# AugmentariumLab/VolumeRenderer

Measured on AMD Instinct MI355X. Metric: Mvoxels/s kd-tree compress+decode, higher is better.
Workload: dtype u8; 1 GPU; 2048x2048x1920 uint8 volume per GPU as 960 bricks of 256x256x128, rm_volume, tolerance 1, maxEpochs 2, VolumeKdtree build + levelCut

## Files before the change

volumerenderer_amd/csrc/brickset.h:

```cpp
#pragma once
#include "kd_common.h"
#include "../../include/vrhip.h"
#include <algorithm>
#include <string>
#include <vector>

namespace vr {

struct Stream2 {
    uint8_t *temp = nullptr;
    uint8_t *codes = nullptr;
    uint8_t *recon[3] = {nullptr, nullptr, nullptr};
    Ctrl *ctrl = nullptr;
    uint8_t *tree = nullptr;
    uint8_t *treeCompact = nullptr;
};

struct Switches {
    bool decodeWalk = false;
    bool decodeFineV1 = false;
    bool decodeQuad = false;
    bool noSkipBlocks = false;
    bool noUniformBlocks = false;
};

#define VR_LOD_SLOTS 4
struct LodSlot {
    int32_t *dev = nullptr;
    int32_t *host = nullptr;
    uint8_t *idxValCut = nullptr;
    uint32_t *decTables = nullptr;
    uint8_t *rankVals = nullptr;
    int64_t *obDev = nullptr;
    int64_t *obHost = nullptr;
    vr_pool_entry *tabHost = nullptr;
    int64_t tabCap = 0;
    hipEvent_t done = nullptr;
    bool pending = false;
};

struct BrickSet {
    int32_t B = 0;
    Switches sw;
    Geom g{};
    TilePlan tile{};
    RegionPlan region{};
    Pyr12Plan pyr12{};
    int32_t D = 0, maxDepth = 0;
    int32_t tolerance = 6, maxEpochs = 5, variant = 0;
    int32_t K = 0;
    int32_t Ds = 0;
    int64_t heapStride = 0;
    int64_t leafStride = 0;
    int64_t codeStride = 0;
    int64_t reconStride = 0;
    bool leafless = false;
    int64_t treeCap = 0;
    int64_t nIdx = 0;

    Stream2 mid, rng;
    uint8_t *mmMin[2] = {nullptr, nullptr}, *mmMax[2] = {nullptr, nullptr};
    unsigned long long *blockErr = nullptr;
    int64_t nErrBlk = 0;
    void *estSumm = nullptr;
    int64_t estSummStride = 0;
    unsigned long long *blockL1 = nullptr;
    uint8_t *blockFlag = nullptr;
    uint8_t *blockFlagR = nullptr;
    uint8_t *blockAlive = nullptr, *blockVal = nullptr;
    unsigned long long *blockSpine = nullptr, *blockSpineR = nullptr;
    uint32_t *chainLut = nullptr;
    uint32_t *blockTot = nullptr, *blockOff = nullptr;
    bool idx64 = false;
    unsigned long long *blockOff64 = nullptr, *idxBase = nullptr;
    int64_t nEmitBlk = 0;
    uint32_t *idxOff = nullptr;
    uint8_t *idxVal = nullptr;
    uint8_t *idxValCut = nullptr;
    uint8_t *fineIdx = nullptr;
    std::vector<uint8_t> fineHas;
    bool fineAll = false;
    uint32_t *decTables = nullptr;
    uint8_t *idxVal3 = nullptr;
    uint32_t *chainTab = nullptr;
    bool chainTabReady = false;
    std::vector<std::vector<uint8_t>> hostTree;
    uint32_t *lut = nullptr;
    bool foreignRange = false;
    uint32_t *spread = nullptr;
    bool generalGeom = false;
    uint32_t *srcIdx = nullptr;
    uint32_t *ownerRank = nullptr;
    uint8_t *ownerSurv = nullptr;
    uint8_t *rankVals = nullptr;

    std::vector<Ctrl> hostCtrl;
    std::vector<int32_t> hostRevertsR;
    uint32_t lutZeroRun = 0;
    bool encoderReady = false;
    bool built = false, hostCtrlValid = false;
    bool gapped = false;
    bool compactValid = false;
    bool compactOnBuild = true;
    int64_t compactCap = 0;
    unsigned long long *brickOff = nullptr;
    int32_t *compactOverflow = nullptr;
    std::vector<unsigned long long> hostBrickOff;
    bool foreign = false;
    std::vector<int64_t> openTreeBytes;
    hipEvent_t ev[8] = {nullptr, nullptr, nullptr, nullptr, nullptr, nullptr, nullptr, nullptr};
    hipStream_t aux = nullptr, auxN[3] = {nullptr, nullptr, nullptr};
    hipEvent_t evFork = nullptr, evJoin = nullptr, evJoinN[3] = {nullptr, nullptr, nullptr};
    int levelLoopStreams = 2;
    unsigned long long *blockErrR = nullptr;
    void *estSummR = nullptr;
    float phasesMs[5] = {0, 0, 0, 0, 0};
// ... 36 lines not shown
```

volumerenderer_amd/csrc/capi.hip:

```cpp
#include "../../include/vrhip.h"
#include "brickset.h"
#include "raymarch.h"
#include <math.h>
#include <stdio.h>
#include <stdlib.h>
#include <string.h>
#include <algorithm>
#include <array>
#include <atomic>
#include <map>
#include <mutex>
#include <new>

using namespace vr;

struct vr_brickset { BrickSet s; };

#define HIPCHK(x) do { hipError_t e_ = (x); if (e_ != hipSuccess) return e_ == hipErrorOutOfMemory ? VR_ERR_OOM : VR_ERR_NO_DEVICE; } while (0)

static bool device_ok()
{
    int n = 0;
    hipError_t e = hipGetDeviceCount(&n);
    if ((e != hipSuccess || n <= 0) && getenv("VRHIP_DEBUG"))
// ... 143 lines not shown
    HIPCHK(hipMalloc(&b.blockAlive, B * (size_t)b.nEmitBlk));
    HIPCHK(hipMalloc(&b.blockVal, B * (size_t)b.nEmitBlk));
    HIPCHK(hipMalloc(&b.blockSpine, B * (size_t)b.nEmitBlk * sizeof(unsigned long long)));
    if (b.variant == VR_VARIANT_MIDRANGE) HIPCHK(hipMalloc(&b.blockSpineR, B * (size_t)b.nEmitBlk * sizeof(unsigned long long)));
    HIPCHK(hipMalloc(&b.chainLut, (260 + 512) * sizeof(uint32_t)));
    HIPCHK(hipMalloc(&b.blockTot, B * (size_t)b.nEmitBlk * sizeof(uint32_t)));
    HIPCHK(hipMalloc(&b.blockOff, B * (size_t)b.nEmitBlk * sizeof(uint32_t)));
    if (b.idx64) {
        HIPCHK(hipMalloc(&b.blockOff64, B * (size_t)b.nEmitBlk * sizeof(unsigned long long)));
        if (!b.idxBase) HIPCHK(hipMalloc(&b.idxBase, B * (size_t)b.nEmitBlk * sizeof(unsigned long long)));
    }
    return VR_OK;
}

static vr_status ensure_encoder_buffers(BrickSet &b)
{
    if (b.encoderReady) return VR_OK;
    const vr_status rc = alloc_encoder_buffers(b);
    if (rc != VR_OK) { (void)hipGetLastError(); free_encoder_buffers(b); return rc; }
    b.encoderReady = true;
    return VR_OK;
}

vr_status vr_brickset_destroy(vr_brickset *h)
{
    if (!h) return VR_OK;
    BrickSet &b = h->s;
    free_lod_slots(&b);
    hipFree(b.errTable);
    free_encoder_buffers(b);
    free_stream2(b.mid);
    free_stream2(b.rng);
    hipFree(b.brickOff); hipFree(b.compactOverflow);
    hipFree(b.idxOff); hipFree(b.idxVal); hipFree(b.idxValCut); hipFree(b.fineIdx); hipFree(b.idxVal3); hipFree(b.chainTab); hipFree(b.decTables); hipFree(b.lut); hipFree(b.spread); hipFree(b.srcIdx); hipFree(b.ownerRank); hipFree(b.ownerSurv); hipFree(b.rankVals);
    for (int i = 0; i < 8; ++i) if (b.ev[i]) hipEventDestroy(b.ev[i]);
    if (b.evFork) hipEventDestroy(b.evFork);
    for (int i = 0; i < 3; ++i) { if (b.evJoinN[i]) hipEventDestroy(b.evJoinN[i]); if (b.auxN[i]) hipStreamDestroy(b.auxN[i]); }
    delete h;
    return VR_OK;
}

static bool pow2(int64_t v) { return v > 0 && (v & (v - 1)) == 0; }

static bool misaligned16(const void *p) { return ((uintptr_t)p & 15) != 0; }

vr_status vr_brickset_create(vr_brickset **out, int32_t num_bricks, const int64_t dims[3], int32_t tolerance,
                             int32_t max_epochs, int32_t variant)
{
    if (!out || !dims || num_bricks <= 0) return VR_ERR_INVALID;
    if (tolerance < 0 || max_epochs < 0 || variant < 0 || variant > 2) return VR_ERR_INVALID;
    for (int k = 0; k < 3; ++k) if (dims[k] <= 0) return VR_ERR_INVALID;
    bool general = !pow2(dims[0]) || !pow2(dims[1]) || !pow2(dims[2]) || dims[0] > 1024 || dims[1] > 1024 || dims[2] > 1024;
    if (dims[0] > (1ll << 20) || dims[1] > (1ll << 20) || dims[2] > (1ll << 20) || dims[0] * dims[1] * dims[2] >= (1ll << 32))
        return VR_ERR_UNSUPPORTED;
    if (!device_ok()) return VR_ERR_NO_DEVICE;
    vr_brickset *h = new (std::nothrow) vr_brickset();
    if (!h) return VR_ERR_OOM;
    BrickSet &b = h->s;
    b.B = num_bricks;
    {
        Switches &w = b.sw;
        w.decodeWalk = getenv("VRHIP_DECODE_WALK") != nullptr;
        w.decodeFineV1 = getenv("VRHIP_DECODE_FINE_V1") != nullptr;
        w.decodeQuad = getenv("VRHIP_DECODE_QUAD") != nullptr;
        w.noSkipBlocks = getenv("VRHIP_NO_SKIP_BLOCKS") != nullptr;
        w.noUniformBlocks = getenv("VRHIP_NO_UNIFORM_BLOCKS") != nullptr;
    }
    make_geom(b.g, dims);
    b.D = b.g.D;
    if (b.D > 31) { delete h; return VR_ERR_UNSUPPORTED; }
    b.idx64 = b.D > 28 || (getenv("VRHIP_FORCE_IDX64") && b.D >= 12);
    if (b.idx64) general = true;
    if (b.idx64 && num_bricks != 1 && b.D > 28) { delete h; return VR_ERR_UNSUPPORTED; }
    b.generalGeom = general;
    b.maxDepth = b.D + VR_CHAIN_LEVELS;
    b.tolerance = tolerance; b.maxEpochs = max_epochs; b.variant = variant;
    b.K = b.D < 6 ? b.D : 6;
    b.Ds = b.D - b.K;
    b.heapStride = (int64_t)1 << (b.D + 1);
    b.leafStride = (int64_t)1 << b.D;
    b.codeStride = ((b.heapStride + 15) / 16) * 4;
    b.reconStride = b.leafStride;
    const int64_t numMax = b.heapStride - 1 + VR_CHAIN_LEVELS * b.leafStride;
    b.treeCap = ((numMax + 15) / 16 + 2) * 4 + 256;
    if (b.D >= 12) {
        const int64_t gappedBytes = ((int64_t)1 << (b.D - 12)) * 2320 * 4 + 256;
        if (gappedBytes > b.treeCap) b.treeCap = gappedBytes;
    }
    b.nIdx = (int64_t)1 << b.Ds;
    make_plans(b.g, b.K, b.generalGeom, b.idx64, b.treeCap, b.tile, b.region, b.pyr12);
    vr_status rc = alloc_stream2(b, b.mid);
    if (rc == VR_OK) {
        hipError_t e = hipMalloc(&b.idxOff, (size_t)b.B * b.nIdx * sizeof(uint32_t));
        if (e == hipSuccess) e = hipMalloc(&b.idxVal, (size_t)b.B * b.nIdx);
        if (e == hipSuccess) e = hipMalloc(&b.idxValCut, (size_t)b.B * b.nIdx);
        if (e == hipSuccess && general) {
            const int grc = build_general_geometry(&b);
            if (grc != 0) e = grc == -3 ? hipErrorOutOfMemory : hipErrorUnknown;
        }
        const auto upload = [](uint32_t *dst, const std::vector<uint32_t> &v) {
            return hipMemcpy(dst, v.data(), v.size() * sizeof(uint32_t), hipMemcpyHostToDevice);
        };
        if (e == hipSuccess) e = hipMalloc(&b.lut, ((size_t)1 << b.K) * sizeof(uint32_t));
        if (e == hipSuccess && !general) e = upload(b.lut, make_lut(b.g, b.K));
        if (e == hipSuccess && !general) e = hipMalloc(&b.spread, (size_t)(b.g.X + b.g.Y + b.g.Z) * sizeof(uint32_t));
        if (e == hipSuccess && !general) e = upload(b.spread, make_spread(b.g));
        for (int i = 0; i < 8 && e == hipSuccess; ++i) e = hipEventCreate(&b.ev[i]);
        if (e != hipSuccess) rc = e == hipErrorOutOfMemory ? VR_ERR_OOM : VR_ERR_NO_DEVICE;
    }
    if (rc != VR_OK) { vr_brickset_destroy(h); return rc; }
    b.hostCtrl.resize(b.B);
    b.openTreeBytes.assign(b.B, -1);
    *out = h;
    return VR_OK;
}

vr_status vr_brickset_set_switch(vr_brickset *h, const char *name, int32_t value)
{
    if (!h || !name) return VR_ERR_INVALID;
    Switches &w = h->s.sw;
    const bool on = value != 0;
    if (!strcmp(name, "decode_walk")) w.decodeWalk = on;
    else if (!strcmp(name, "decode_fine_v1")) w.decodeFineV1 = on;
    else if (!strcmp(name, "decode_quad")) w.decodeQuad = on;
    else if (!strcmp(name, "no_skip_blocks")) w.noSkipBlocks = on;
    else if (!strcmp(name, "no_uniform_blocks")) w.noUniformBlocks = on;
    else return VR_ERR_INVALID;
    return VR_OK;
}

vr_status vr_brickset_set_compaction(vr_brickset *h, int32_t on_build)
{
    if (!h) return VR_ERR_INVALID;
    h->s.compactOnBuild = on_build != 0;
    return VR_OK;
}

vr_status vr_debug_set(const char *name, int32_t value)
{
    if (!name) return VR_ERR_INVALID;
    if (!strcmp(name, "skip_grid_v1")) { vr::g_skipGridV1.store(value ? 1 : 0); return VR_OK; }
    if (!strcmp(name, "reslice_tile_w")) {
        if (value != 8 && value != 16 && value != 64) return VR_ERR_INVALID;
        vr::g_resliceTileLog2.store(value == 8 ? 3 : (value == 16 ? 4 : 6));
        return VR_OK;
    }
    if (!strcmp(name, "hist_plain")) { vr::g_histPlain.store(value ? 1 : 0); return VR_OK; }
    return VR_ERR_INVALID;
}

vr_status vr_brickset_set_error_tolerance(vr_brickset *h, int32_t tol)
{
    if (!h || tol < 0) return VR_ERR_INVALID;
    h->s.tolerance = tol;
    return VR_OK;
}
vr_status vr_brickset_set_max_epochs(vr_brickset *h, int32_t e)
{
    if (!h || e < 0) return VR_ERR_INVALID;
// ... 1008 lines not shown
```

volumerenderer_amd/csrc/kd_decode.hip:

```cpp
#include "brickset.h"
#include <stdio.h>
#include <algorithm>
#include <stdlib.h>
#include <string.h>

namespace vr {

int launch_status(const char *what)
{
    hipError_t e = hipGetLastError();
    if (e == hipSuccess) return 0;
    if (getenv("VRHIP_DEBUG")) fprintf(stderr, "[vrhip] %s: %s\n", what, hipGetErrorString(e));
    return -1;
}

struct Box3 { int lo[3], hi[3]; };
__device__ __forceinline__ int split_axis(const Box3 &b, int depth, bool &more)
{
    const long long e0 = b.hi[0] - b.lo[0], e1 = b.hi[1] - b.lo[1], e2 = b.hi[2] - b.lo[2];
    more = e0 * e1 * e2 > 1;
    int sd = depth % 3, i = 0;
    while (more && (b.hi[sd] - b.lo[sd]) == 1) sd = (depth + ++i) % 3;
    return sd;
}
// ... 938 lines not shown
#define RG_REGX (16 * RG_WAVES)
#define RG_BLK_WORDS 1028
#define RG_RING_MASK (RG_NP * 256 - 1)
static_assert(RG_REGX == VR_RG_REGX, "region_plan (host_plan.cpp) lays the regions out for this x extent");
static_assert(RG_NP >= 4 && (RG_NP & (RG_NP - 1)) == 0, "the side-cars of the next region are staged in ring slots 2 and 3: at least four pieces, a power of two");

struct RegionArgs {
    const uint8_t *tree;
    int64_t treeCap;
    const uint32_t *idxOff;
    const uint8_t *idxVal;
    const uint8_t *fine;
    const uint8_t *val3;
    int64_t nIdx;
    const Ctrl *ctrls;
    uint8_t *out;
    const uint32_t *spread;
    int X, Y;
    int64_t voxels;
    int D, cut;
    int lrx, lry;
    int jx;
    uint32_t lanePos;
    uint32_t parkP[4];
    uint32_t parkS;
    uint32_t gAddr[4];
    uint32_t gByte;
    uint32_t gOut[8];
    uint32_t xRead[2];
    uint32_t blkX, blkY, blkZ;
    int nreg;
    const int32_t *list, *cuts;
    const int64_t *obase;
};

__device__ __forceinline__ uint32_t wave_incl_scan_max_dpp(uint32_t v)
{
    v = max(v, dpp_u32<0x111, 0xf>(0, v));
    v = max(v, dpp_u32<0x112, 0xf>(0, v));
    v = max(v, dpp_u32<0x114, 0xf>(0, v));
    v = max(v, dpp_u32<0x118, 0xf>(0, v));
    v = max(v, dpp_u32<0x142, 0xa>(0, v));
    v = max(v, dpp_u32<0x143, 0xc>(0, v));
    return v;
}

__device__ __forceinline__ void rg_barrier()
{
    asm volatile("s_waitcnt lgkmcnt(0)\n\ts_barrier" ::: "memory");
}

struct RegionShared {
    uint32_t leafA[1024];
    uint32_t chainB[64];
    int d4[4], d5[4];
    uint32_t buf[RG_WAVES * RG_BLK_WORDS];
    uint32_t ring[RG_WAVES][RG_NP * 256 + 4];
};

__device__ __forceinline__ uint32_t rg_pair(uint32_t y, uint32_t yh, uint32_t dead3, int Vp, const RegionShared &sm, uint32_t &used)
{
    const uint32_t c5 = (y & 3u) | dead3;
    const int V5 = med3i(Vp + *(const int *)((const char *)sm.d5 + (c5 << 2)), 0, 255);
    const bool pr = c5 == 3u;
    const uint32_t keep = pr ? 0u : ~0u;
    const uint32_t yl1 = y >> 2;
// ... 24 lines not shown
{
    const uint32_t b = (pw >> 7) & 30u;
    const int V3 = (int)(pw & 255u);
    const uint32_t dead = ((pw >> 24) & 1u) - 1u;
    const uint32_t lo = __builtin_amdgcn_alignbit(w1, w0, b), hi = __builtin_amdgcn_alignbit(w2, w1, b),
                   hh = __builtin_amdgcn_alignbit(w3, w2, b);
    const uint32_t c4 = __builtin_amdgcn_ubfe(lo, p0, 2) | (dead & 3u);
    const int V4 = med3i(V3 + *(const int *)((const char *)sm.d4 + (c4 << 2)), 0, 255);
    const uint32_t dead3 = c4 == 3u ? 3u : 0u;
    uint32_t used1, used2;
    const uint32_t b01 = rg_pair(__builtin_amdgcn_alignbit(hi, lo, p1), __builtin_amdgcn_alignbit(hh, hi, p1), dead3, V4, sm, used1);
    const uint32_t p2 = p1 + used1;
    const bool q = p2 >= 32u;
    const uint32_t A_ = q ? hi : lo, B_ = q ? hh : hi, C_ = q ? 0u : hh;
    const uint32_t b23 = rg_pair(__builtin_amdgcn_alignbit(B_, A_, p2), __builtin_amdgcn_alignbit(C_, B_, p2), dead3, V4, sm, used2);
    return b01 | (b23 << 16);
}

__device__ __forceinline__ void rg_vm_wait(uint32_t n)
{
    switch (n < 24u ? n : 24u) {
#define RG_W(k) case k: asm volatile("s_waitcnt vmcnt(" #k ")" ::: "memory"); break;
    RG_W(0) RG_W(1) RG_W(2) RG_W(3) RG_W(4) RG_W(5) RG_W(6) RG_W(7) RG_W(8) RG_W(9) RG_W(10) RG_W(11) RG_W(12)
    RG_W(13) RG_W(14) RG_W(15) RG_W(16) RG_W(17) RG_W(18) RG_W(19) RG_W(20) RG_W(21) RG_W(22) RG_W(23) RG_W(24)
#undef RG_W
    }
}

#define RG_DMA(SUFFIX, gptr, ldsByte) do { uint32_t keep_; \
    asm volatile("s_mov_b32 %0, m0\n\ts_mov_b32 m0, %2\n\ts_nop 0\n\tglobal_load_lds_" SUFFIX " %1, off\n\ts_mov_b32 m0, %0" \
                 : "=&s"(keep_) : "v"(gptr), "s"(ldsByte) : "memory"); } while (0)

#define RG_IDXD 3

__global__ void __launch_bounds__(64 * RG_WAVES, RG_MINW)
k_decode_region(RegionArgs a)
{
    struct Shared {
        RegionShared t;
        uint32_t idxOff[RG_WAVES][RG_IDXD][64];
        uint32_t idxVal[RG_WAVES][RG_IDXD][16];
        uint32_t blkTab[3][64];
    };
    __shared__ __attribute__((aligned(16))) Shared smw;
    RegionShared &sm = smw.t;
    const int wave = __builtin_amdgcn_readfirstlane((int)(threadIdx.x >> 6)), lane = threadIdx.x & 63;
    const int brick = lod_brick(a.list, blockIdx.y);
    const int G = (int)gridDim.x;
    const int nreg = a.nreg;
    int rid = (int)blockIdx.x;
    if (rid >= nreg) return;
    {
        const int cut = lod_cut(a.cuts, brick, a.cut);
        const uint8_t *dmap = a.ctrls[brick].distanceMap;
        const int t = threadIdx.x;
        if (t < 192) {
            const int ax = t >> 6, v = t & 63;
            const uint32_t pos = ax == 0 ? a.blkX : (ax == 1 ? a.blkY : a.blkZ);
            uint32_t r = 0;
#pragma unroll
            for (int k = 0; k < 6; ++k) r |= (((uint32_t)v >> k) & 1u) << ((pos >> (5 * k)) & 31u);
            smw.blkTab[ax][v] = r;
        }
        const auto compose = [](int tok0, bool withCode, int d0, const int *dist, int n, uint32_t key) {
            int A = 0, LO = 0, HI = 255;
            bool go = true;
            if (withCode) {
                go = tok0 != 3;
                const int dl = tok0 == 1 ? d0 : (tok0 == 2 ? -d0 : 0);
                A += dl; LO = min(max(LO + dl, 0), 255); HI = min(max(HI + dl, 0), 255);
            }
            for (int q = 0; q < n; ++q) {
                const int tok = (int)((key >> (2 * q)) & 3u);
                go = go && tok != 3;
// ... 31 lines not shown
    uint32_t qlow = 0;
#pragma unroll
    for (int i = 0; i < 6; ++i) qlow |= (((uint32_t)lane >> i) & 1u) << ((a.lanePos >> (4 * i)) & 15u);
    const uint32_t g = qlow & 15u;
    const uint32_t ownN = g == 0u ? 4u : (uint32_t)(__ffs((int)g) - 1);
    const uint32_t p0 = 2u * ownN, p1 = p0 + 2u;
    uint32_t addrL = 0, byteL = 0, outL = 0;
#pragma unroll
    for (int i = 0; i < 8; ++i) {
        if (i >= 6 - RG_LW && i < 8 - RG_LW) continue;
        const bool on = i < 6 - RG_LW ? ((lane >> (RG_LW + i)) & 1) != 0 : ((wave >> (i - (8 - RG_LW))) & 1) != 0;
        addrL ^= on ? (a.gAddr[i >> 1] >> (16 * (i & 1))) & 0xFFFFu : 0u;
        byteL |= on ? (a.gByte >> (4 * i)) & 15u : 0u;
        outL += on ? a.gOut[i] : 0u;
    }
    uint32_t ops = 0;
    uint32_t markIdx[RG_IDXD];
    uint32_t markP[RG_NP];
    const auto mark_of_idx = [&](int slot) { uint32_t m = 0;
#pragma unroll
        for (int i = 0; i < RG_IDXD; ++i) m = slot == i ? markIdx[i] : m;
        return m; };
    const auto mark_of_piece = [&](uint32_t p) { uint32_t m = 0;
#pragma unroll
        for (int i = 0; i < RG_NP; ++i) m = (p & (RG_NP - 1)) == (uint32_t)i ? markP[i] : m;
        return m; };
#pragma unroll
    for (int i = 0; i < RG_NP; ++i) markP[i] = 0;
    const auto index_of = [&](int r) -> int64_t {
        const uint32_t rx = (uint32_t)r & ((1u << a.lrx) - 1u), ry = ((uint32_t)r >> a.lrx) & ((1u << a.lry) - 1u), rz = (uint32_t)r >> (a.lrx + a.lry);
        const uint32_t blk = smw.blkTab[0][rx * (uint32_t)RG_WAVES + (uint32_t)wave] | smw.blkTab[1][ry] | smw.blkTab[2][rz];
        return (int64_t)brick * a.nIdx + ((int64_t)blk << 6);
    };
    const auto request_index = [&](int r, int slot) {
        const int64_t io = index_of(r);
        RG_DMA("dword", a.idxOff + io + lane, idxOffLds + (uint32_t)slot * 256u);
        if (lane < 16) RG_DMA("dword", (const uint32_t *)(a.idxVal + io) + lane, idxValLds + (uint32_t)slot * 64u);
        ops += 2;
#pragma unroll
        for (int i = 0; i < RG_IDXD; ++i) markIdx[i] = slot == i ? ops : markIdx[i];
    };
    const auto issue_piece = [&](uint32_t wbase, uint32_t p) {
        const uint32_t w = wbase + 256u * p + 4u * (uint32_t)lane;
        if (w + 4u <= capWords) RG_DMA("dwordx4", W + w, ringLds + (p & (RG_NP - 1)) * 1024u);
        ++ops;
#pragma unroll
        for (int i = 0; i < RG_NP; ++i) markP[i] = (p & (RG_NP - 1)) == (uint32_t)i ? ops : markP[i];
    };
    unsigned long long liveMask = 0ull;
    uint32_t wbase = 0, totalPieces = 0, issued = 0, markSide = 0, offC = VR_IDX_DEAD, valC = 0;
    const auto stage = [&](int r, int slot) {
        rg_vm_wait(ops - mark_of_idx(slot));
        offC = smw.idxOff[wave][slot][lane];
        valC = (smw.idxVal[wave][slot][lane >> 2] >> (8 * (lane & 3))) & 255u;
        const bool liveL = offC != VR_IDX_DEAD;
        liveMask = __ballot(liveL);
        wbase = 0; totalPieces = 0; issued = 0;
        if (liveMask == 0ull) return;
        const int firstL = __ffsll((long long)liveMask) - 1, lastL = 63 - __clzll((long long)liveMask);
        const uint32_t firstOff = (uint32_t)__builtin_amdgcn_readlane((int)offC, firstL), lastOff = (uint32_t)__builtin_amdgcn_readlane((int)offC, lastL);
        wbase = (firstOff >> 4) & ~3u;
        const uint32_t tp = ((((lastOff + 575u + 15u) >> 4) - wbase) + 255u) >> 8;
        totalPieces = min(tp, (capWords - wbase + 255u) >> 8);
        for (uint32_t p = 0; p < 2u && p < totalPieces; ++p) { issue_piece(wbase, p); ++issued; }
        const int64_t io = index_of(r);
        RG_DMA("dwordx4", a.fine + (io + lane) * 16, ringLds + 3u * 1024u);
        if (lane < 32) RG_DMA("dwordx4", a.val3 + io * 8 + lane * 16, ringLds + 2u * 1024u);
        ops += 2;
        markSide = ops;
    };
#pragma unroll
    for (int d = 0; d < RG_IDXD; ++d) markIdx[d] = 0;
#pragma unroll
    for (int d = 0; d < RG_IDXD; ++d) if (rid + d * G < nreg) request_index(rid + d * G, d);
    stage(rid, 0);
    int slot = 0;
    for (; rid < nreg; rid += G) {
        if (liveMask == 0ull) {
            const uint32_t rep = valC * 0x01010101u;
#pragma unroll
            for (int gg = 0; gg < 16; ++gg) buf[laneTerm ^ ((a.parkP[gg >> 2] >> (8 * (gg & 3))) & 255u)] = rep;
            if (rid + RG_IDXD * G < nreg) request_index(rid + RG_IDXD * G, slot);
        } else {
            const bool liveL = offC != VR_IDX_DEAD;
            rg_vm_wait(ops - markSide);
            const uint4 cv = *(const uint4 *)(ringW + 768 + 4 * lane);
            const uint2 sv = *(const uint2 *)(ringW + 512 + 2 * lane);
            const uint32_t cw[4] = {cv.x, cv.y, cv.z, cv.w}, sw2[2] = {sv.x, sv.y};
            const bool stepDead = ((uint32_t)(liveMask >> (lane & 60)) & 15u) == 0u;
            const uint32_t deadW = stepDead ? valC * 0x01010101u : valC;
            uint32_t run = liveL ? offC - wbase * 16u : 0u;
#pragma unroll
            for (int gg = 0; gg < 16; ++gg) {
                const uint32_t cgg = (cw[gg >> 2] >> (8 * (gg & 3))) & 255u;
                const int own = gg == 0 ? 4 : (gg & 1 ? 0 : (gg & 2 ? 1 : (gg & 4 ? 2 : 3)));
                const uint32_t vgg = (sw2[gg >> 3] >> (8 * ((gg >> 1) & 3))) & 255u;
                const uint32_t w = vgg | (run << 8) | ((uint32_t)(own - (int)cgg) & 0x01000000u);
                buf[laneTerm ^ ((a.parkP[gg >> 2] >> (8 * (gg & 3))) & 255u)] = liveL ? w : deadW;
                run += cgg;
            }
            const uint32_t mEnd = wave_incl_scan_max_dpp(liveL ? run : 0u);
            asm volatile("s_waitcnt lgkmcnt(0)" ::: "memory");
            for (uint32_t p = 2; p < (uint32_t)RG_NP && p < totalPieces; ++p) { issue_piece(wbase, p); ++issued; }
            if (rid + RG_IDXD * G < nreg) request_index(rid + RG_IDXD * G, slot);
            uint32_t guardNext = RG_NP;
            uint32_t landed = 0;
#pragma unroll 1
            for (int t = 0; t < 8; ++t) {
                const uint32_t nib = ((uint32_t)(liveMask >> (8 * t))) & 255u;
                if (nib == 0u) continue;
                const uint32_t endTok = (uint32_t)__builtin_amdgcn_readlane((int)mEnd, 8 * t + 7);
                const uint32_t need = (((endTok + 15u) >> 4) + 255u) >> 8;
// ... 170 lines not shown
        common(t, out, obase);
        t.jx = p.jx; t.jy = p.jy; t.jz = p.jz;
        t.tilesX = p.tilesX; t.tilesY = p.tilesY; t.tilesZ = p.tilesZ; t.ltx = p.ltx; t.lty = p.lty;
        memcpy(t.kqBit, p.kqBit, sizeof(t.kqBit));
        t.g = bs->g; t.Ds = bs->Ds; t.idxValCut = cutVals; t.spread = bs->spread; t.fine = bs->fineIdx; t.val3 = bs->idxVal3;
        return t;
    };
    const auto lane_args = [&](const unsigned long long *idxBase, const uint32_t *lut, uint8_t *dst, const int64_t *dstBase) {
        DecodeArgs a;
        common(a, dst, dstBase);
        a.idxBase = idxBase; a.nBase = idxBase ? bs->nEmitBlk : 0; a.lut = lut; a.g = bs->g; a.K = bs->K; a.Ds = bs->Ds; a.idxValCut = cutVals;
        return a;
    };
    switch (k) {
    case DecodeKernel::GENERAL: {
        if (!lod && !bs->rankVals && hipMalloc(&bs->rankVals, (size_t)bs->B * bs->leafStride * 2) != hipSuccess) return -3;
        uint8_t *rankVals = lod ? lod->rankVals : bs->rankVals;
        const DecodeArgs a = lane_args(bs->idx64 ? bs->idxBase : nullptr, nullptr, rankVals, nullptr);
        hipLaunchKernelGGL(k_decode_lane<true>, dim3((unsigned)((bs->nIdx + 63) / 64), rows), dim3(64), 0, st, a);
        hipLaunchKernelGGL(k_owner_gather, dim3((unsigned)((bs->g.voxels + 255) / 256), rows), dim3(256), 0, st,
                           (const uint16_t *)rankVals, bs->leafStride, bs->ownerRank, bs->ownerSurv, bs->g.voxels, out, list, obase);
        break;
    }
    case DecodeKernel::REGION: {
        const RegionPlan &p = bs->region;
        RegionArgs r;
        r.X = p.X; r.Y = p.Y; r.voxels = p.voxels; r.lrx = p.lrx; r.lry = p.lry; r.jx = p.jx;
        r.lanePos = p.lanePos; r.parkS = p.parkS; r.gByte = p.gByte;
        memcpy(r.parkP, p.parkP, sizeof(r.parkP)); memcpy(r.gAddr, p.gAddr, sizeof(r.gAddr));
        memcpy(r.gOut, p.gOut, sizeof(r.gOut)); memcpy(r.xRead, p.xRead, sizeof(r.xRead));
        r.blkX = p.blkX; r.blkY = p.blkY; r.blkZ = p.blkZ; r.nreg = p.nreg;
        common(r, out, obase);
        r.fine = bs->fineIdx; r.val3 = bs->idxVal3; r.spread = bs->spread;
        unsigned wgs = (unsigned)((r.nreg + RG_PER - 1) / RG_PER);
        if ((int64_t)wgs * rows < 2048) wgs = (unsigned)std::min<int64_t>(r.nreg, (2048 + rows - 1) / rows);
        hipLaunchKernelGGL(k_decode_region, dim3(wgs, rows), dim3(64 * RG_WAVES), 0, st, r);
        break;
    }
    case DecodeKernel::QUAD: {
        TileArgs t = tile_args();
        const int ntiles = t.tilesX * t.tilesY * t.tilesZ;
        const int levels = cut - bs->D < 0 ? 0 : (cut - bs->D > VR_CHAIN_LEVELS ? VR_CHAIN_LEVELS : cut - bs->D);
        if (!bs->chainTab && hipMalloc(&bs->chainTab, (size_t)(VR_CHAIN_LEVELS + 1) * QD_CHAIN_ENTRIES * 4) != hipSuccess) return -3;
        if (!bs->chainTabReady) {
            for (int lv = 0; lv <= VR_CHAIN_LEVELS; ++lv)
                hipLaunchKernelGGL(k_chain_table, dim3(QD_CHAIN_ENTRIES / 256), dim3(256), 0, st, lv, bs->chainTab + (size_t)lv * QD_CHAIN_ENTRIES);
            if (hipStreamSynchronize(st) != hipSuccess) return -1;
            bs->chainTabReady = true;
        }
        t.tables = bs->chainTab + (lod ? (size_t)0 : (size_t)levels * QD_CHAIN_ENTRIES);
        const int per = QD_WAVES * QD_TPW;
        hipLaunchKernelGGL(k_decode_quad, dim3((unsigned)((ntiles + per - 1) / per), rows), dim3(64 * QD_WAVES), 0, st, t);
        break;
    }
    case DecodeKernel::FINE:
    case DecodeKernel::TILE: {
        TileArgs t = tile_args();
        const int ntiles = t.tilesX * t.tilesY * t.tilesZ;
        const bool useFine = k == DecodeKernel::FINE;
        if (useFine && !lod && !bs->decTables && hipMalloc(&bs->decTables, (size_t)bs->B * FD_TABLE_WORDS * 4) != hipSuccess) return -3;
        uint32_t *decTables = lod ? lod->decTables : bs->decTables;
        t.tables = decTables;
        if (useFine) {
            hipLaunchKernelGGL(k_fine_tables, dim3(rows), dim3(256), 0, st, bs->mid.ctrl, bs->D, bs->Ds, cut, decTables, list, cuts);
            hipLaunchKernelGGL(k_decode_fine, dim3((unsigned)((ntiles + FD_WAVES - 1) / FD_WAVES), rows),
                               dim3(64 * FD_WAVES), 0, st, t);
// ... 209 lines not shown
```

volumerenderer_amd/csrc/kd_encode.hip:

```cpp
#include "brickset.h"
#include <math.h>
#include <stdio.h>
#include <stdlib.h>
#include <string.h>

namespace vr {

#define FILL_NODES_PER_BLOCK 1024
#define EMIT_RANKS_PER_BLOCK 256

template <bool FROM_VOXELS>
__global__ void __launch_bounds__(256)
k_pyramid(Geom g, int dLeaf, int L, const uint8_t *__restrict__ vox, const uint8_t *__restrict__ inMin,
          const uint8_t *__restrict__ inMax, int64_t inStride, uint8_t *__restrict__ temp, int64_t heapStride,
          uint8_t *__restrict__ tempRange, uint8_t *__restrict__ outMin, uint8_t *__restrict__ outMax,
          int64_t outStride, const uint32_t *__restrict__ srcIdx)
{
    __shared__ uint8_t smn[2][1024], smx[2][1024];
    const int brick = blockIdx.y;
    const uint32_t n = 1u << L;
    const uint32_t base = blockIdx.x << L;
    uint8_t *T = temp + (int64_t)brick * heapStride;
    uint8_t *TR = tempRange ? tempRange + (int64_t)brick * heapStride : nullptr;
    for (uint32_t i = threadIdx.x; i < n; i += blockDim.x) {
// ... 1324 lines not shown
    if (lane == 63) shWave[w] = incl;
    __syncthreads();
    const uint32_t s0 = shWave[0], s1 = shWave[1], s2 = shWave[2], s3 = shWave[3];
    __syncthreads();
    total = s0 + s1 + s2 + s3;
    const uint32_t woff = w == 0 ? 0u : (w == 1 ? s0 : (w == 2 ? s0 + s1 : s0 + s1 + s2));
    return woff + incl - v;
}

#define PE_WORDS 2320
#define PE_TOKENS (PE_WORDS * 16)

struct PruneEmitArgs {
    int D, tol, maxDepth;
    Ctrl *ctrls;
    uint8_t *temp;
    uint8_t *codes;
    int64_t heapStride, codeStride, leafStride;
    ReconBufs rb;
    uint32_t *subTok;
    int64_t nEmitBlk;
    unsigned long long *blockL1;
    const uint32_t *chainLut;
    uint32_t *idxOff;
    int64_t nIdx;
    uint32_t *fineIdx;
    Ctrl *ctrlsR;
    uint8_t *tempR, *codesR;
    ReconBufs rbR;
    uint8_t *gap, *gapR;
    int64_t treeCap;
    SkipBlocks sk, skR;
    int uniformBlocks;
};

__device__ __forceinline__ void pe_put(uint32_t *W, uint32_t bitpos, unsigned long long v, int ntok)
{
    if (ntok <= 0) return;
    const uint32_t sh = bitpos & 31u, w = bitpos >> 5;
    const unsigned long long lo = v << sh;
    atomicOr(&W[w], (uint32_t)lo);
    if ((uint32_t)(lo >> 32)) atomicOr(&W[w + 1], (uint32_t)(lo >> 32));
    const uint32_t hi = sh ? (uint32_t)(v >> (64u - sh)) : 0u;
    if (hi) atomicOr(&W[w + 2], hi);
}

template <class LUT>
__device__ __forceinline__ void pe_leaf_table(uint32_t T2, vr_s16x2 dl, uint32_t cl2, uint32_t tol2, const LUT &lut, vr_s16x2 &mxB,
                                                  uint32_t &m, uint32_t &sg, uint32_t &act, uint32_t &Lb, uint32_t &nt,
                                                  uint32_t &bothMask, int j)
{
    const vr_s16x2 mm = pk_abs(dl);
    m = pk_u(mm);
    sg = pk_u(dl >> 15);
    mxB = __builtin_elementwise_max(mxB, mm);
    const uint32_t lt = pk_u((mm - pk_s(tol2)) >> 15);
    const uint32_t isz = pk_u((pk_s(cl2) - pk_s(0x00010001u)) >> 15), is3 = pk_u((pk_s(0x00020002u) - pk_s(cl2)) >> 15);
    const uint32_t newp = isz & lt;
    const uint32_t pruned = newp | is3;
    const uint32_t lcode = cl2 | (newp & 0x00030003u);
    bothMask |= ((pruned & (pruned >> 16)) & 1u) << (2 * j);
    const vr_s16x2 lim = __builtin_elementwise_min(pk_s(T2), pk_s(T2 ^ 0x00FF00FFu));
    const uint32_t viol = pk_u((lim - mm) >> 15);
    const uint32_t e0 = lut(pk_u(dl) & 511u), e1 = lut((pk_u(dl) >> 16) & 511u);
    const uint32_t useL = ~pruned & ~viol;
    const uint32_t ch2 = __builtin_amdgcn_perm(e1, e0, 0x07060302u);
// ... 438 lines not shown
    }
    __syncthreads();
    for (int i = t; i < PEC_BOXES * 16; i += 256) {
        const int b = i >> 4, l = i & 15;
        if ((res[b][0] & 15u) != 1u) continue;
        const uint32_t blk = blk0 + (uint32_t)b;
        *(uint4 *)(a.idxOff + (int64_t)brick * a.nIdx + ((int64_t)blk << 6) + l * 4) = make_uint4(VR_IDX_DEAD, VR_IDX_DEAD, VR_IDX_DEAD, VR_IDX_DEAD);
        if (l < 4) a.blockL1[(int64_t)brick * a.nEmitBlk + (size_t)blk * 4 + l] = stat_pack(0, 0, 0);
        if (l == 0) {
            cset3(Cb, ((int64_t)1 << (D - 12)) + blk);
            a.subTok[(int64_t)brick * a.nEmitBlk + blk] = 1;
            *((uint32_t *)(a.gap + (int64_t)brick * a.treeCap) + (size_t)blk * PE_WORDS) = 3u;
        }
    }
    const int jmin = t ? 8 - (__ffs(t) - 1) : 0;
    for (int b = 0; b < PEC_BOXES; ++b) {
        const uint32_t r0 = res[b][0];
        if ((r0 & 15u) != 2u) continue;
        const uint32_t blk = blk0 + (uint32_t)b, base = blk << 12;
        const int P = (int)((r0 >> 4) & 15u);
        const uint32_t changed = (r0 >> 8) & 0xFFFu, uc = res[b][1], LbL = res[b][2] & 0xFFFFu, ntL = res[b][2] >> 16;
        const uint32_t len8 = res[b][3] & 0xFFFFu, len10 = res[b][3] >> 16, tot = res[b][4];
        const uint32_t nw = min((tot + 15u) / 16u + 1u, (uint32_t)PE_WORDS);
        for (uint32_t i = t; i < nw; i += 256u) W[i] = 0;
        if (t < 12) Pc[t] = 0;
        if (t >= 1 && t < 64) {
            const int h = t * 4, lq = 31 - __clz(h);
            if ((changed >> lq) & 1u) Cb[(((int64_t)1 << (D - 12 + lq)) + ((int64_t)blk << lq) + (h - (1 << lq))) >> 2] = 0xFFu;
        }
        if (t >= 1 && t < 4) {
            const int lq = 31 - __clz(t);
            if ((changed >> lq) & 1u) cset3(Cb, ((int64_t)1 << (D - 12 + lq)) + ((int64_t)blk << lq) + (t - (1 << lq)));
        }
        if (t == 0) a.subTok[(int64_t)brick * a.nEmitBlk + blk] = tot;
        if (t < 4) {
            const uint32_t fe = res[b][5] & 0xFFFFu, eB = res[b][5] >> 16;
            a.blockL1[(int64_t)brick * a.nEmitBlk + (size_t)blk * 4 + t] = stat_pack((unsigned long long)fe * 1024ull, (int)eB, (int)fe);
        }
        if ((r0 >> 20) & 1u) atomicAdd(&c.zeroRun, 4);
        __syncthreads();
        const int top = P < 7 ? P : 7;
        const int ns = jmin <= top ? top - jmin + 1 : 0;
        uint32_t pos = P >= 8 ? (uint32_t)t * len8 : 0u;
        for (int lq = 0; lq <= top; ++lq) pos += ((uint32_t)t + (1u << (8 - lq)) - 1u) >> (8 - lq);
        uint32_t bitpos = 2u * pos;
        pe_put(W, bitpos, (unsigned long long)((uc >> (2 * jmin)) & ((1u << (2 * ns)) - 1u)), ns);
        bitpos += 2u * (uint32_t)ns;
        if (P >= 11 && t < 8) {
            const uint32_t a4 = (uc >> 16) & 3u, a3 = (uc >> 18) & 3u, a2 = (uc >> 20) & 3u, a1 = (uc >> 22) & 3u;
            unsigned long long H = a1;
            int Hn = 1;
            if (a1 != 3u) { H |= ((unsigned long long)LbL << 2) | ((unsigned long long)LbL << (2 + 2 * ntL)); Hn = 1 + 2 * (int)ntL; }
            const int pn = (int)((0x01020103u >> (4 * t)) & 15u);
            const int pre = (0x76644330u >> (4 * t)) & 15;
            const uint32_t pb = t == 0 ? a4 | (a3 << 2) | (a2 << 4) : (t == 4 ? a3 | (a2 << 2) : a2);
            pe_put(Pc, 2u * (uint32_t)(pre + t * Hn), (unsigned long long)(pn ? pb : 0u) | (H << (2 * pn)), pn + Hn);
        }
        if (P >= 8 && P < 11) {
            const uint32_t a4 = (uc >> 16) & 3u, a3 = (uc >> 18) & 3u, a2 = (uc >> 20) & 3u;
            const uint32_t pc = P == 8 ? a4 : (P == 9 ? a4 | (a3 * 0x14u) : a4 | (a3 * 0x104u) | (a2 * 0x1450u));
            pe_put(W, bitpos, (unsigned long long)pc, (int)len8);
        }
        if (P >= 11) {
            __syncthreads();
            const uint32_t b1 = bitpos + 2u * len8 - 1u, w0 = bitpos >> 5, w1 = b1 >> 5, sh = bitpos & 31u;
            uint32_t lo = 0;
            for (uint32_t w = w0; w <= w1; ++w) {
// ... 724 lines not shown
    if (parts > 1) parts = 1 + ensure_aux(bs, parts - 1);
    if (parts > 1) {
        hipEventRecord(bs->evFork, st);
        for (int p = 1; p < parts; ++p) {
            const int b0 = (int)((int64_t)B * p / parts), b1 = (int)((int64_t)B * (p + 1) / parts);
            hipStreamWaitEvent(bs->auxN[p - 1], bs->evFork, 0);
            compress_stream(bs, bs->mid, bs->auxN[p - 1], cMin, cMax, rootStride, sk, bs->blockErr, bs->estSumm, b0, b1 - b0);
            hipEventRecord(bs->evJoinN[p - 1], bs->auxN[p - 1]);
        }
        compress_stream(bs, bs->mid, st, cMin, cMax, rootStride, sk, bs->blockErr, bs->estSumm, 0, (int)((int64_t)B / parts));
        for (int p = 1; p < parts; ++p) hipStreamWaitEvent(st, bs->evJoinN[p - 1], 0);
    } else
    compress_stream(bs, bs->mid, st, cMin, cMax, rootStride, sk, bs->blockErr, bs->estSumm);
    if (forkR) hipStreamWaitEvent(st, bs->evJoin, 0);
    else if (mr) compress_stream(bs, bs->rng, st, cMin, cMax, rootStride, skR, bs->blockErr, bs->estSumm);
    hipEventRecord(bs->ev[2], st);
    dbg_sync(st, "compress");
    hipLaunchKernelGGL(k_chain_lut, dim3(1), dim3(256), 0, st, bs->tolerance, bs->maxDepth - D, bs->chainLut);
    ReconBufs rb{{bs->mid.recon[0], bs->mid.recon[1], bs->mid.recon[2]}};
    ReconBufs rbR{{bs->rng.recon[0], bs->rng.recon[1], bs->rng.recon[2]}};
    int pruneFrom = D - 1;
    bs->fineHas.assign((size_t)B, 0);
    fine_has_changed(*bs);
    if (fused) {
        PruneEmitArgs pa;
        pa.sk = sk; pa.skR = skR;
        pa.D = D; pa.tol = bs->tolerance; pa.maxDepth = bs->maxDepth; pa.ctrls = bs->mid.ctrl;
        pa.temp = bs->mid.temp; pa.codes = bs->mid.codes;
        pa.heapStride = bs->heapStride; pa.codeStride = bs->codeStride; pa.leafStride = bs->reconStride;
        pa.rb = rb; pa.subTok = bs->blockOff; pa.nEmitBlk = bs->nEmitBlk; pa.blockL1 = bs->blockL1;
        pa.chainLut = bs->chainLut; pa.idxOff = bs->idxOff; pa.nIdx = bs->nIdx;
        if (!bs->fineIdx && hipMalloc(&bs->fineIdx, (size_t)B * bs->nIdx * 16) != hipSuccess) return -3;
        if (!bs->idxVal3 && hipMalloc(&bs->idxVal3, (size_t)B * bs->nIdx * 8) != hipSuccess) return -3;
        pa.fineIdx = (uint32_t *)bs->fineIdx;
        pa.ctrlsR = mr ? bs->rng.ctrl : nullptr; pa.tempR = mr ? bs->rng.temp : nullptr; pa.codesR = mr ? bs->rng.codes : nullptr;
        pa.rbR = rbR;
        pa.gap = bs->mid.tree; pa.gapR = mr ? bs->rng.tree : nullptr; pa.treeCap = bs->treeCap;
        const dim3 peGrid((unsigned)((int64_t)1 << (D - 12)), B);
        pa.uniformBlocks = skipOn && bs->leafless && !mr && !bs->sw.noUniformBlocks;
        if (pa.uniformBlocks)
            hipLaunchKernelGGL(k_prune_emit12_const, dim3((unsigned)cdiv((int64_t)1 << (D - 12), PEC_BOXES), B), dim3(256), 0, st, pa);
        if (bs->leafless) {
            hipLaunchKernelGGL((k_prune_emit12<false, true>), peGrid, dim3(256), 0, st, pa);
            if (mr) hipLaunchKernelGGL((k_prune_emit12<true, true>), peGrid, dim3(256), 0, st, pa);
        } else {
            hipLaunchKernelGGL((k_prune_emit12<false, false>), peGrid, dim3(256), 0, st, pa);
            if (mr) hipLaunchKernelGGL((k_prune_emit12<true, false>), peGrid, dim3(256), 0, st, pa);
        }
        pruneFrom = D - 13;
        bs->fineHas.assign((size_t)B, 1);
        fine_has_changed(*bs);
    } else
        hipLaunchKernelGGL(k_prune_leaf, dim3(cdiv((int64_t)1 << D, 256), B), dim3(256), 0, st, D, bs->tolerance,
                           bs->mid.ctrl, bs->mid.temp, bs->mid.codes, mr ? bs->rng.codes : nullptr, bs->heapStride,
                           bs->codeStride, rb, bs->reconStride, bs->maxDepth, bs->blockL1, bs->nEmitBlk);
    for (int d = pruneFrom; d >= 0; --d)
        hipLaunchKernelGGL(k_prune_level, dim3(cdiv((int64_t)1 << d, 256), B), dim3(256), 0, st, d, bs->mid.ctrl, bs->mid.codes,
                           mr ? bs->rng.codes : nullptr, bs->codeStride);
    hipLaunchKernelGGL(k_fix_chain_distances, dim3(B), dim3(64), 0, st, D, bs->maxDepth, bs->mid.ctrl,
                       mr ? bs->rng.ctrl : nullptr);
    hipEventRecord(bs->ev[3], st);
    dbg_sync(st, "prune");
    EmitArgs a;
    fill_emit_args(bs, a);
    const int64_t nblk = cdiv((int64_t)1 << D, fused ? 4096 : EMIT_RANKS_PER_BLOCK);
    if (fused) hipLaunchKernelGGL(k_block_alive, dim3(cdiv(nblk, 256), B), dim3(256), 0, st, a, nblk, 12);
    else hipLaunchKernelGGL(k_emit_count, dim3((unsigned)nblk, B), dim3(EMIT_RANKS_PER_BLOCK), 0, st, a);
// ... 25 lines not shown
```

Baseline: 277,600 Mvoxels/s.

## Flag uniform boxes in encoder and shortcut their region decode

The const prune-emit kernel now marks each uniform 4096-voxel box in a new per-brick boxUniform array. The region decoder fetches that flag alongside the index values. For flagged boxes it loads only a single piece and fine/val3 word, decodes one value and broadcasts it. This cuts DMA traffic and per-voxel decode work for uniform regions, at the cost of a memset and an extra flag load per index request.

```diff
diff --git a/volumerenderer_amd/csrc/brickset.h b/volumerenderer_amd/csrc/brickset.h
--- a/volumerenderer_amd/csrc/brickset.h
+++ b/volumerenderer_amd/csrc/brickset.h
@@ -22,6 +22,7 @@
     bool decodeQuad = false;
     bool noSkipBlocks = false;
     bool noUniformBlocks = false;
+    bool noUniformDecode = false;
 };
 
 #define VR_LOD_SLOTS 4
@@ -82,6 +83,7 @@
     bool fineAll = false;
     uint32_t *decTables = nullptr;
     uint8_t *idxVal3 = nullptr;
+    uint32_t *boxUniform = nullptr;
     uint32_t *chainTab = nullptr;
     bool chainTabReady = false;
     std::vector<std::vector<uint8_t>> hostTree;
diff --git a/volumerenderer_amd/csrc/capi.hip b/volumerenderer_amd/csrc/capi.hip
--- a/volumerenderer_amd/csrc/capi.hip
+++ b/volumerenderer_amd/csrc/capi.hip
@@ -199,7 +199,7 @@
     free_stream2(b.mid);
     free_stream2(b.rng);
     hipFree(b.brickOff); hipFree(b.compactOverflow);
-    hipFree(b.idxOff); hipFree(b.idxVal); hipFree(b.idxValCut); hipFree(b.fineIdx); hipFree(b.idxVal3); hipFree(b.chainTab); hipFree(b.decTables); hipFree(b.lut); hipFree(b.spread); hipFree(b.srcIdx); hipFree(b.ownerRank); hipFree(b.ownerSurv); hipFree(b.rankVals);
+    hipFree(b.idxOff); hipFree(b.idxVal); hipFree(b.idxValCut); hipFree(b.fineIdx); hipFree(b.idxVal3); hipFree(b.boxUniform); hipFree(b.chainTab); hipFree(b.decTables); hipFree(b.lut); hipFree(b.spread); hipFree(b.srcIdx); hipFree(b.ownerRank); hipFree(b.ownerSurv); hipFree(b.rankVals);
     for (int i = 0; i < 8; ++i) if (b.ev[i]) hipEventDestroy(b.ev[i]);
     if (b.evFork) hipEventDestroy(b.evFork);
     for (int i = 0; i < 3; ++i) { if (b.evJoinN[i]) hipEventDestroy(b.evJoinN[i]); if (b.auxN[i]) hipStreamDestroy(b.auxN[i]); }
@@ -232,6 +232,7 @@
         w.decodeQuad = getenv("VRHIP_DECODE_QUAD") != nullptr;
         w.noSkipBlocks = getenv("VRHIP_NO_SKIP_BLOCKS") != nullptr;
         w.noUniformBlocks = getenv("VRHIP_NO_UNIFORM_BLOCKS") != nullptr;
+        w.noUniformDecode = getenv("VRHIP_NO_UNIFORM_DECODE") != nullptr;
     }
     make_geom(b.g, dims);
     b.D = b.g.D;
@@ -292,6 +293,7 @@
     else if (!strcmp(name, "decode_quad")) w.decodeQuad = on;
     else if (!strcmp(name, "no_skip_blocks")) w.noSkipBlocks = on;
     else if (!strcmp(name, "no_uniform_blocks")) w.noUniformBlocks = on;
+    else if (!strcmp(name, "no_uniform_decode")) w.noUniformDecode = on;
     else return VR_ERR_INVALID;
     return VR_OK;
 }
diff --git a/volumerenderer_amd/csrc/kd_decode.hip b/volumerenderer_amd/csrc/kd_decode.hip
--- a/volumerenderer_amd/csrc/kd_decode.hip
+++ b/volumerenderer_amd/csrc/kd_decode.hip
@@ -994,6 +994,7 @@
     int nreg;
     const int32_t *list, *cuts;
     const int64_t *obase;
+    const uint32_t *uni;
 };
 
 __device__ __forceinline__ uint32_t wave_incl_scan_max_dpp(uint32_t v)
@@ -1084,6 +1085,7 @@
                  : "=&s"(keep_) : "v"(gptr), "s"(ldsByte) : "memory"); } while (0)
 
 #define RG_IDXD 3
+#define RG_IDXV 20
 
 __global__ void __launch_bounds__(64 * RG_WAVES, RG_MINW)
 k_decode_region(RegionArgs a)
@@ -1091,7 +1093,7 @@
     struct Shared {
         RegionShared t;
         uint32_t idxOff[RG_WAVES][RG_IDXD][64];
-        uint32_t idxVal[RG_WAVES][RG_IDXD][16];
+        uint32_t idxVal[RG_WAVES][RG_IDXD][RG_IDXV];
         uint32_t blkTab[3][64];
     };
     __shared__ __attribute__((aligned(16))) Shared smw;
@@ -1189,40 +1191,46 @@
         const uint32_t blk = smw.blkTab[0][rx * (uint32_t)RG_WAVES + (uint32_t)wave] | smw.blkTab[1][ry] | smw.blkTab[2][rz];
         return (int64_t)brick * a.nIdx + ((int64_t)blk << 6);
     };
+    const int idxLanes = a.uni ? 17 : 16;
     const auto request_index = [&](int r, int slot) {
         const int64_t io = index_of(r);
         RG_DMA("dword", a.idxOff + io + lane, idxOffLds + (uint32_t)slot * 256u);
-        if (lane < 16) RG_DMA("dword", (const uint32_t *)(a.idxVal + io) + lane, idxValLds + (uint32_t)slot * 64u);
+        const uint32_t *vp = a.uni && lane == 16 ? a.uni + (io >> 6) : (const uint32_t *)(a.idxVal + io) + lane;
+        if (lane < idxLanes) RG_DMA("dword", vp, idxValLds + (uint32_t)slot * (4u * RG_IDXV));
         ops += 2;
 #pragma unroll
         for (int i = 0; i < RG_IDXD; ++i) markIdx[i] = slot == i ? ops : markIdx[i];
     };
-    const auto issue_piece = [&](uint32_t wbase, uint32_t p) {
+    const auto issue_piece = [&](uint32_t wbase, uint32_t p, int nl = 64) {
         const uint32_t w = wbase + 256u * p + 4u * (uint32_t)lane;
-        if (w + 4u <= capWords) RG_DMA("dwordx4", W + w, ringLds + (p & (RG_NP - 1)) * 1024u);
+        if (w + 4u <= capWords && lane < nl) RG_DMA("dwordx4", W + w, ringLds + (p & (RG_NP - 1)) * 1024u);
         ++ops;
 #pragma unroll
         for (int i = 0; i < RG_NP; ++i) markP[i] = (p & (RG_NP - 1)) == (uint32_t)i ? ops : markP[i];
     };
     unsigned long long liveMask = 0ull;
     uint32_t wbase = 0, totalPieces = 0, issued = 0, markSide = 0, offC = VR_IDX_DEAD, valC = 0;
+    bool uniC = false;
     const auto stage = [&](int r, int slot) {
         rg_vm_wait(ops - mark_of_idx(slot));
         offC = smw.idxOff[wave][slot][lane];
         valC = (smw.idxVal[wave][slot][lane >> 2] >> (8 * (lane & 3))) & 255u;
         const bool liveL = offC != VR_IDX_DEAD;
         liveMask = __ballot(liveL);
-        wbase = 0; totalPieces = 0; issued = 0;
+        wbase = 0; totalPieces = 0; issued = 0; uniC = false;
         if (liveMask == 0ull) return;
+        uniC = a.uni && (liveMask & 1ull) != 0ull && __builtin_amdgcn_readfirstlane((int)smw.idxVal[wave][slot][16]) != 0;
         const int firstL = __ffsll((long long)liveMask) - 1, lastL = 63 - __clzll((long long)liveMask);
         const uint32_t firstOff = (uint32_t)__builtin_amdgcn_readlane((int)offC, firstL), lastOff = (uint32_t)__builtin_amdgcn_readlane((int)offC, lastL);
         wbase = (firstOff >> 4) & ~3u;
         const uint32_t tp = ((((lastOff + 575u + 15u) >> 4) - wbase) + 255u) >> 8;
         totalPieces = min(tp, (capWords - wbase + 255u) >> 8);
-        for (uint32_t p = 0; p < 2u && p < totalPieces; ++p) { issue_piece(wbase, p); ++issued; }
+        if (uniC) totalPieces = min(totalPieces, 1u);
+        const int pieceLanes = uniC ? 2 : 64, fineLanes = uniC ? 1 : 64, val3Lanes = uniC ? 1 : 32;
+        for (uint32_t p = 0; p < 2u && p < totalPieces; ++p) { issue_piece(wbase, p, pieceLanes); ++issued; }
         const int64_t io = index_of(r);
-        RG_DMA("dwordx4", a.fine + (io + lane) * 16, ringLds + 3u * 1024u);
-        if (lane < 32) RG_DMA("dwordx4", a.val3 + io * 8 + lane * 16, ringLds + 2u * 1024u);
+        if (lane < fineLanes) RG_DMA("dwordx4", a.fine + (io + lane) * 16, ringLds + 3u * 1024u);
+        if (lane < val3Lanes) RG_DMA("dwordx4", a.val3 + io * 8 + lane * 16, ringLds + 2u * 1024u);
         ops += 2;
         markSide = ops;
     };
@@ -1235,6 +1243,16 @@
     for (; rid < nreg; rid += G) {
         if (liveMask == 0ull) {
             const uint32_t rep = valC * 0x01010101u;
+#pragma unroll
+            for (int gg = 0; gg < 16; ++gg) buf[laneTerm ^ ((a.parkP[gg >> 2] >> (8 * (gg & 3))) & 255u)] = rep;
+            if (rid + RG_IDXD * G < nreg) request_index(rid + RG_IDXD * G, slot);
+        } else if (uniC) {
+            rg_vm_wait(ops - markSide);
+            const uint32_t c0 = ringW[768] & 255u, v0 = ringW[512] & 255u;
+            const uint32_t run = (uint32_t)__builtin_amdgcn_readfirstlane((int)offC) - wbase * 16u;
+            const uint32_t pw = v0 | (run << 8) | ((4u - c0) & 0x01000000u);
+            const uint32_t *r0 = ringW + ((pw >> 12) & RG_RING_MASK);
+            const uint32_t rep = (rg_quad(pw, r0[0], r0[1], r0[2], r0[3], 8u, 10u, sm) & 255u) * 0x01010101u;
 #pragma unroll
             for (int gg = 0; gg < 16; ++gg) buf[laneTerm ^ ((a.parkP[gg >> 2] >> (8 * (gg & 3))) & 255u)] = rep;
             if (rid + RG_IDXD * G < nreg) request_index(rid + RG_IDXD * G, slot);
@@ -1471,6 +1489,7 @@
         r.blkX = p.blkX; r.blkY = p.blkY; r.blkZ = p.blkZ; r.nreg = p.nreg;
         common(r, out, obase);
         r.fine = bs->fineIdx; r.val3 = bs->idxVal3; r.spread = bs->spread;
+        r.uni = bs->foreign || rangeStream || bs->sw.noUniformDecode ? nullptr : bs->boxUniform;
         unsigned wgs = (unsigned)((r.nreg + RG_PER - 1) / RG_PER);
         if ((int64_t)wgs * rows < 2048) wgs = (unsigned)std::min<int64_t>(r.nreg, (2048 + rows - 1) / rows);
         hipLaunchKernelGGL(k_decode_region, dim3(wgs, rows), dim3(64 * RG_WAVES), 0, st, r);
diff --git a/volumerenderer_amd/csrc/kd_encode.hip b/volumerenderer_amd/csrc/kd_encode.hip
--- a/volumerenderer_amd/csrc/kd_encode.hip
+++ b/volumerenderer_amd/csrc/kd_encode.hip
@@ -1380,6 +1380,7 @@
     int64_t treeCap;
     SkipBlocks sk, skR;
     int uniformBlocks;
+    uint32_t *boxUniform;
 };
 
 __device__ __forceinline__ void pe_put(uint32_t *W, uint32_t bitpos, unsigned long long v, int ntok)
@@ -1884,7 +1885,10 @@
             const int lq = 31 - __clz(t);
             if ((changed >> lq) & 1u) cset3(Cb, ((int64_t)1 << (D - 12 + lq)) + ((int64_t)blk << lq) + (t - (1 << lq)));
         }
-        if (t == 0) a.subTok[(int64_t)brick * a.nEmitBlk + blk] = tot;
+        if (t == 0) {
+            a.subTok[(int64_t)brick * a.nEmitBlk + blk] = tot;
+            a.boxUniform[(int64_t)brick * a.sk.nBlk + blk] = 1u;
+        }
         if (t < 4) {
             const uint32_t fe = res[b][5] & 0xFFFFu, eB = res[b][5] >> 16;
             a.blockL1[(int64_t)brick * a.nEmitBlk + (size_t)blk * 4 + t] = stat_pack((unsigned long long)fe * 1024ull, (int)eB, (int)fe);
@@ -2675,7 +2679,10 @@
         pa.chainLut = bs->chainLut; pa.idxOff = bs->idxOff; pa.nIdx = bs->nIdx;
         if (!bs->fineIdx && hipMalloc(&bs->fineIdx, (size_t)B * bs->nIdx * 16) != hipSuccess) return -3;
         if (!bs->idxVal3 && hipMalloc(&bs->idxVal3, (size_t)B * bs->nIdx * 8) != hipSuccess) return -3;
-        pa.fineIdx = (uint32_t *)bs->fineIdx;
+        const size_t boxBytes = (size_t)B * ((size_t)1 << (D - 12)) * sizeof(uint32_t);
+        if (!bs->boxUniform && hipMalloc(&bs->boxUniform, boxBytes) != hipSuccess) return -3;
+        if (hipMemsetAsync(bs->boxUniform, 0, boxBytes, st) != hipSuccess) return -1;
+        pa.fineIdx = (uint32_t *)bs->fineIdx; pa.boxUniform = bs->boxUniform;
         pa.ctrlsR = mr ? bs->rng.ctrl : nullptr; pa.tempR = mr ? bs->rng.temp : nullptr; pa.codesR = mr ? bs->rng.codes : nullptr;
         pa.rbR = rbR;
         pa.gap = bs->mid.tree; pa.gapR = mr ? bs->rng.tree : nullptr; pa.treeCap = bs->treeCap;
```

New measurement: 280,700 Mvoxels/s (median of 6 runs). +1.1%, better.
